# PeihaoChen/WS-MGMap

Hardware: AMD Instinct MI355X
Metric: policy steps/sec (fwd+bwd), CMA batch=8 seq=64 (higher is better)
Workload: dtype bf16

## Files before the change

ws-mgmap_amd/csrc/wsmg_conv_win_wgrad.hip:

```cpp
#include <stdlib.h>

#include "wsmg_conv_tile.h"

namespace {

struct WinWgradArgs {
  const bf16_t* x;
  const bf16_t* dy;
  float* dw;
  int64_t slab;
  int B, H, W, OH, OW, tiles_y, tiles_x, groups;
  unsigned x_bytes, dy_bytes;
};

constexpr int K = 8, S = 2, P = 3, TH = 5, TW = 25;
constexpr int WC = (TW - 1) * S + K;
constexpr int PC = WC / S;
constexpr int PITCH = 192;
constexpr int XROW = S * PC * PITCH;
constexpr int X_BYTES = TH * XROW;
constexpr int NPX = 128;
constexpr int D_BYTES = NPX * PITCH;
constexpr int DPER = NPX * 8 / 256;

__global__ __launch_bounds__(256, 2) void conv_win_wgrad_kernel(WinWgradArgs a) {
  extern __shared__ __attribute__((aligned(16))) unsigned char lds[];
  unsigned char* const xs = lds;
  unsigned char* const ds = lds + X_BYTES;
  const int tid = threadIdx.x, lane = tid & 63, wave = tid >> 6;
  const int xcd = blockIdx.x & 7, li_ = blockIdx.x >> 3;
  const int ky = li_ & 7, grp = xcd + 8 * (li_ >> 3);
  const int tpi = a.tiles_y * a.tiles_x;
  const int ntiles = a.B * tpi;
  const __amdgpu_buffer_rsrc_t xr = make_rsrc(a.x, a.x_bytes), dr = make_rsrc(a.dy, a.dy_bytes);

  constexpr int XPER2 = 2 * TH;
  const int wc0 = tid >> 3, pch = tid & 7;
  const bool has1 = tid < (WC - 32) * 8;
  const int xl0 = ((wc0 & 1) * PC + (wc0 >> 1)) * PITCH + pch * 16;
  const int xl1 = xl0 + 16 * PITCH;
  int doff[DPER];
#pragma unroll
  for (int j = 0; j < DPER; ++j) {
    const int q = wc0 + 32 * j;
    const int qr = (q * 41) >> 10;
    doff[j] = q < TH * TW ? ((qr * a.OW + q - qr * TW) * 64) * 2 + pch * 16 : -1;
  }
  u32x4 rx[XPER2], rd[DPER];
  auto gload = [&](int tile) {
    const int b = tile / tpi, t = tile - b * tpi;
    const int ty = t / a.tiles_x;
    const int oy0 = ty * TH, ox0 = (t - ty * a.tiles_x) * TW;
    const int ix0 = ox0 * S - P, iyb = oy0 * S - P + ky;
    const bool live = tile < ntiles;
    const int c0 = ix0 + wc0, c1 = c0 + 32;
    const bool ok0 = (unsigned)c0 < (unsigned)a.W, ok1 = has1 && (unsigned)c1 < (unsigned)a.W;
    const int cb0 = c0 * 128 + pch * 16, cb1 = cb0 + 32 * 128;
#pragma unroll
    for (int j = 0; j < TH; ++j) {
      const int iy = iyb + j * S;
      const bool rowok = live && (unsigned)iy < (unsigned)a.H;
      const int base = ((b * a.H + iy) * a.W) * 128;
      rx[2 * j] = buf_load16(xr, (rowok && ok0) ? base + cb0 : (int)0x80000000);
      rx[2 * j + 1] = buf_load16(xr, (rowok && ok1) ? base + cb1 : (int)0x80000000);
    }
    const bool whole = live && oy0 + TH <= a.OH && ox0 + TW <= a.OW;
    const int dbase = (((b * a.OH + oy0) * a.OW + ox0) * 64) * 2;
#pragma unroll
    for (int j = 0; j < DPER; ++j) {
      bool ok = whole && doff[j] >= 0;
      if (!whole && live && doff[j] >= 0) {
        const int q = wc0 + 32 * j, qr = (q * 41) >> 10;
        ok = oy0 + qr < a.OH && ox0 + q - qr * TW < a.OW;
      }
      rd[j] = buf_load16(dr, ok ? dbase + doff[j] : (int)0x80000000);
    }
  };
  auto lstore = [&]() {
#pragma unroll
    for (int j = 0; j < TH; ++j) {
      *reinterpret_cast<u32x4*>(xs + j * XROW + xl0) = rx[2 * j];
      if (has1) *reinterpret_cast<u32x4*>(xs + j * XROW + xl1) = rx[2 * j + 1];
    }
#pragma unroll
    for (int j = 0; j < DPER; ++j) *reinterpret_cast<u32x4*>(ds + (wc0 + 32 * j) * PITCH + pch * 16) = rd[j];
  };

  const int li = lane & 15, q4 = li >> 2, p4 = li & 3;
  const int half16 = (lane >> 4) & 1, h = lane >> 5;
  const int chan_off = (half16 * 16 + p4 * 4) * 2;
  const int l0 = 8 * h + q4;
  auto xoff = [&](int c, int s2) {
    int p = 16 * c + l0 + 4 * s2;
    p = p < TH * TW ? p : TH * TW - 1;
    const int jr = (p * 41) >> 10;
    return jr * XROW + (p - jr * TW) * PITCH + chan_off;
  };
  const unsigned char* const a_base = ds + (8 * h + q4) * PITCH + chan_off;
  const int kx0 = 2 * wave;
  const int tapoff0 = ((kx0 & 1) * PC + (kx0 >> 1)) * PITCH, tapoff1 = (((kx0 + 1) & 1) * PC + ((kx0 + 1) >> 1)) * PITCH;

  f32x16 acc[2][4];
#pragma unroll
  for (int t = 0; t < 2; ++t)
#pragma unroll
    for (int v = 0; v < 4; ++v)
#pragma unroll
      for (int g = 0; g < 16; ++g) acc[t][v][g] = 0.f;

  int tile = grp;
  if (tile >= ntiles) return;
  gload(tile);
  lstore();
  __syncthreads();
  struct Frag { bf16x8 a[2], b[4]; };
  auto fload = [&](int c, Frag& f) {
#pragma unroll
    for (int t = 0; t < 2; ++t) {
      const bf16x4 l = tr_read(a_base + 64 * t + (16 * c) * PITCH), hh = tr_read(a_base + 64 * t + (16 * c + 4) * PITCH);
      f.a[t] = __builtin_shufflevector(l, hh, 0, 1, 2, 3, 4, 5, 6, 7);
    }
    const int x0 = xoff(c, 0), x1 = xoff(c, 1);
#pragma unroll
    for (int v = 0; v < 4; ++v) {
      const int to = (v >> 1) ? tapoff1 : tapoff0;
      const bf16x4 l = tr_read(xs + x0 + to + 64 * (v & 1)), hh = tr_read(xs + x1 + to + 64 * (v & 1));
      f.b[v] = __builtin_shufflevector(l, hh, 0, 1, 2, 3, 4, 5, 6, 7);
    }
  };
  for (; tile < ntiles; tile += a.groups) {
    gload(tile + a.groups);
    Frag cur, nxt;
    fload(0, cur);
#pragma unroll
    for (int c = 0; c < 8; ++c) {
      __builtin_amdgcn_sched_barrier(0);
      if (c + 1 < 8) fload(c + 1, nxt);
#pragma unroll
      for (int v = 0; v < 4; ++v)
#pragma unroll
        for (int t = 0; t < 2; ++t) acc[t][v] = __builtin_amdgcn_mfma_f32_32x32x16_bf16(cur.a[t], cur.b[v], acc[t][v], 0, 0, 0);
      if (c + 1 < 8) {
#pragma unroll
        for (int i = 0; i < 4; ++i) {
          __builtin_amdgcn_sched_group_barrier(0x008, 1, 0);
          __builtin_amdgcn_sched_group_barrier(0x100, 2, 0);
          __builtin_amdgcn_sched_group_barrier(0x008, 1, 0);
          __builtin_amdgcn_sched_group_barrier(0x100, 1, 0);
        }
      }
      __builtin_amdgcn_sched_barrier(0);
      if (c + 1 < 8) cur = nxt;
    }
    __syncthreads();
    lstore();
    __syncthreads();
  }

  const int r = lane & 31;
#pragma unroll
  for (int v = 0; v < 4; ++v) {
    const int tap = ky * K + kx0 + (v >> 1);
    const int ci = 32 * (v & 1) + r;
#pragma unroll
    for (int t = 0; t < 2; ++t)
#pragma unroll
      for (int g = 0; g < 16; ++g) {
        const int co = 32 * t + (g & 3) + 8 * (g >> 2) + 4 * h;
        float* const q = a.dw + (size_t)grp * a.slab + ((size_t)co * (K * K) + tap) * 64 + ci;
        if (a.slab) *q = acc[t][v][g];
        else atomicAdd(q, acc[t][v][g]);
      }
  }
}

}

static bool winw_fits(int B, int H, int W, int Cin, int Cout, int KH, int KW, int stride, int pad, int OH, int OW) {
  if (Cin != 64 || Cout != 64 || KH != 8 || KW != 8 || stride != 2 || pad != 3) return false;
  return !((size_t)B * H * W * 128 >= (1ull << 31) || (size_t)B * OH * OW * 128 >= (1ull << 31));
}
static int winw_groups(int B, int OH, int OW) {
  const int ntiles = B * ((OH + TH - 1) / TH) * ((OW + TW - 1) / TW);
  int groups = 64;
  if (groups > ntiles) groups = ntiles;
  return (groups + 7) / 8 * 8;
}

int wsmg_conv_win_wgrad_splits(int B, int H, int W, int Cin, int Cout, int KH, int KW, int stride, int pad, int OH, int OW) {
  return winw_fits(B, H, W, Cin, Cout, KH, KW, stride, pad, OH, OW) ? winw_groups(B, OH, OW) : 0;
}

int wsmg_conv_win_wgrad_bf16(const void* x, const void* dy, float* dw_ohwi, long long slab_floats, int B, int H, int W, int Cin, int Cout,
                             int KH, int KW, int stride, int pad, int OH, int OW, hipStream_t s) {
  if (!winw_fits(B, H, W, Cin, Cout, KH, KW, stride, pad, OH, OW)) return WSMG_EINVAL;
  WinWgradArgs a{(const bf16_t*)x, (const bf16_t*)dy, dw_ohwi, (int64_t)slab_floats, B, H, W, OH, OW, (OH + TH - 1) / TH, (OW + TW - 1) / TW, 0,
                 (unsigned)((size_t)B * H * W * 128), (unsigned)((size_t)B * OH * OW * 128)};
  const int groups = winw_groups(B, OH, OW);
  a.groups = groups;
  static bool attr = false;
  if (!attr) {
    hipError_t e = hipFuncSetAttribute(reinterpret_cast<const void*>(conv_win_wgrad_kernel), hipFuncAttributeMaxDynamicSharedMemorySize,
                                       X_BYTES + D_BYTES);
    if (e != hipSuccess) return (int)e;
    attr = true;
  }
  hipLaunchKernelGGL(conv_win_wgrad_kernel, dim3((unsigned)(8 * groups)), dim3(256), X_BYTES + D_BYTES, s, a);
  WSMG_RETURN_LAUNCH();
}
```

Before: 51600.

## Restructure window wgrad kernel: 512-thread blocks sharing x rows, double-buffered LDS pipeline

Each block now runs 8 waves covering two kernel rows (ky and ky+2), so the staged input rows are shared and the grid shrinks from 8 to 4 blocks per group. The LDS layout is split into channel planes with padding in place of a 192-byte pitch. A double-buffered LDS scheme interleaves the next tile's global loads and LDS stores with the MFMA loop, cutting the per-tile pair of barriers to one. The cost is higher LDS use per block and heavier scheduling constraints, which may lower occupancy. Blocks that have no tile no longer exit early when slab mode is on, so they still write their zero slab.

```diff
diff --git a/ws-mgmap_amd/csrc/wsmg_conv_win_wgrad.hip b/ws-mgmap_amd/csrc/wsmg_conv_win_wgrad.hip
--- a/ws-mgmap_amd/csrc/wsmg_conv_win_wgrad.hip
+++ b/ws-mgmap_amd/csrc/wsmg_conv_win_wgrad.hip
@@ -16,74 +16,74 @@
 constexpr int K = 8, S = 2, P = 3, TH = 5, TW = 25;
 constexpr int WC = (TW - 1) * S + K;
 constexpr int PC = WC / S;
-constexpr int PITCH = 192;
-constexpr int XROW = S * PC * PITCH;
-constexpr int X_BYTES = TH * XROW;
+constexpr int WR = TH + 1;
+constexpr int ENT = 64;
+constexpr int XCH = PC * ENT + 64;
+constexpr int XPAR = 2 * XCH;
+constexpr int XROW = S * XPAR;
+constexpr int X_BYTES = WR * XROW;
 constexpr int NPX = 128;
-constexpr int D_BYTES = NPX * PITCH;
-constexpr int DPER = NPX * 8 / 256;
-
-__global__ __launch_bounds__(256, 2) void conv_win_wgrad_kernel(WinWgradArgs a) {
+constexpr int DCH = NPX * ENT + 64;
+constexpr int D_BYTES = 2 * DCH;
+constexpr int PARK = X_BYTES + D_BYTES;
+constexpr int BUF = PARK + 64 * 16;
+constexpr int LDS_BYTES = 2 * BUF;
+constexpr int NPIECE = WR + 2;
+constexpr int OOB = (int)0x80000000;
+
+__global__ __launch_bounds__(512) void conv_win_wgrad_kernel(WinWgradArgs a) {
   extern __shared__ __attribute__((aligned(16))) unsigned char lds[];
-  unsigned char* const xs = lds;
-  unsigned char* const ds = lds + X_BYTES;
-  const int tid = threadIdx.x, lane = tid & 63, wave = tid >> 6;
+  const int tid = threadIdx.x, lane = tid & 63, wave = __builtin_amdgcn_readfirstlane(tid >> 6);
   const int xcd = blockIdx.x & 7, li_ = blockIdx.x >> 3;
-  const int ky = li_ & 7, grp = xcd + 8 * (li_ >> 3);
+  const int role = li_ & 3, grp = xcd + 8 * (li_ >> 2);
+  const int ky_lo = (role & 1) + 4 * (role >> 1);
   const int tpi = a.tiles_y * a.tiles_x;
   const int ntiles = a.B * tpi;
   const __amdgpu_buffer_rsrc_t xr = make_rsrc(a.x, a.x_bytes), dr = make_rsrc(a.dy, a.dy_bytes);
 
-  constexpr int XPER2 = 2 * TH;
-  const int wc0 = tid >> 3, pch = tid & 7;
-  const bool has1 = tid < (WC - 32) * 8;
-  const int xl0 = ((wc0 & 1) * PC + (wc0 >> 1)) * PITCH + pch * 16;
-  const int xl1 = xl0 + 16 * PITCH;
-  int doff[DPER];
-#pragma unroll
-  for (int j = 0; j < DPER; ++j) {
-    const int q = wc0 + 32 * j;
+  const bool hasx = wave < 7;
+  const int wc = tid >> 3, pch = tid & 7;
+  const int plane = pch >> 2, pbyte = (pch & 3) * 16;
+  const int xl = hasx ? (wc & 1) * XPAR + plane * XCH + (wc >> 1) * ENT + pbyte : PARK + lane * 16;
+  const int xrs = hasx ? XROW : 0;
+  int dl[2], doff[2];
+#pragma unroll
+  for (int j = 0; j < 2; ++j) {
+    const int q = wc + 64 * j;
     const int qr = (q * 41) >> 10;
+    dl[j] = X_BYTES + plane * DCH + q * ENT + pbyte;
     doff[j] = q < TH * TW ? ((qr * a.OW + q - qr * TW) * 64) * 2 + pch * 16 : -1;
   }
-  u32x4 rx[XPER2], rd[DPER];
-  auto gload = [&](int tile) {
+  int t_row0 = 0, t_bH = 0, t_cb = 0, t_dbase = 0;
+  bool t_okx = false, t_okd[2] = {false, false};
+  auto prep = [&](int tile) {
     const int b = tile / tpi, t = tile - b * tpi;
     const int ty = t / a.tiles_x;
     const int oy0 = ty * TH, ox0 = (t - ty * a.tiles_x) * TW;
-    const int ix0 = ox0 * S - P, iyb = oy0 * S - P + ky;
     const bool live = tile < ntiles;
-    const int c0 = ix0 + wc0, c1 = c0 + 32;
-    const bool ok0 = (unsigned)c0 < (unsigned)a.W, ok1 = has1 && (unsigned)c1 < (unsigned)a.W;
-    const int cb0 = c0 * 128 + pch * 16, cb1 = cb0 + 32 * 128;
-#pragma unroll
-    for (int j = 0; j < TH; ++j) {
-      const int iy = iyb + j * S;
-      const bool rowok = live && (unsigned)iy < (unsigned)a.H;
-      const int base = ((b * a.H + iy) * a.W) * 128;
-      rx[2 * j] = buf_load16(xr, (rowok && ok0) ? base + cb0 : (int)0x80000000);
-      rx[2 * j + 1] = buf_load16(xr, (rowok && ok1) ? base + cb1 : (int)0x80000000);
-    }
-    const bool whole = live && oy0 + TH <= a.OH && ox0 + TW <= a.OW;
-    const int dbase = (((b * a.OH + oy0) * a.OW + ox0) * 64) * 2;
-#pragma unroll
-    for (int j = 0; j < DPER; ++j) {
-      bool ok = whole && doff[j] >= 0;
-      if (!whole && live && doff[j] >= 0) {
-        const int q = wc0 + 32 * j, qr = (q * 41) >> 10;
-        ok = oy0 + qr < a.OH && ox0 + q - qr * TW < a.OW;
-      }
-      rd[j] = buf_load16(dr, ok ? dbase + doff[j] : (int)0x80000000);
-    }
-  };
-  auto lstore = [&]() {
-#pragma unroll
-    for (int j = 0; j < TH; ++j) {
-      *reinterpret_cast<u32x4*>(xs + j * XROW + xl0) = rx[2 * j];
-      if (has1) *reinterpret_cast<u32x4*>(xs + j * XROW + xl1) = rx[2 * j + 1];
-    }
-#pragma unroll
-    for (int j = 0; j < DPER; ++j) *reinterpret_cast<u32x4*>(ds + (wc0 + 32 * j) * PITCH + pch * 16) = rd[j];
+    const int c0 = ox0 * S - P + wc;
+    t_okx = hasx && live && (unsigned)c0 < (unsigned)a.W;
+    t_cb = c0 * 128 + pch * 16;
+    t_bH = b * a.H;
+    t_row0 = oy0 * S - P + ky_lo;
+    t_dbase = (((b * a.OH + oy0) * a.OW + ox0) * 64) * 2;
+#pragma unroll
+    for (int j = 0; j < 2; ++j) {
+      const int q = wc + 64 * j, qr = (q * 41) >> 10;
+      t_okd[j] = live && doff[j] >= 0 && oy0 + qr < a.OH && ox0 + q - qr * TW < a.OW;
+    }
+  };
+  auto loadp = [&](int p) -> u32x4 {
+    if (p < WR) {
+      const int iy = t_row0 + p * S;
+      const bool ok = t_okx && (unsigned)iy < (unsigned)a.H;
+      return buf_load16(xr, ok ? ((t_bH + iy) * a.W) * 128 + t_cb : OOB);
+    }
+    return buf_load16(dr, t_okd[p - WR] ? t_dbase + doff[p - WR] : OOB);
+  };
+  u32x4 rp[NPIECE];
+  auto storep = [&](int p, int buf) {
+    *reinterpret_cast<u32x4*>(lds + buf + (p < WR ? xl + p * xrs : dl[p - WR])) = rp[p];
   };
 
   const int li = lane & 15, q4 = li >> 2, p4 = li & 3;
@@ -94,11 +94,11 @@
     int p = 16 * c + l0 + 4 * s2;
     p = p < TH * TW ? p : TH * TW - 1;
     const int jr = (p * 41) >> 10;
-    return jr * XROW + (p - jr * TW) * PITCH + chan_off;
-  };
-  const unsigned char* const a_base = ds + (8 * h + q4) * PITCH + chan_off;
-  const int kx0 = 2 * wave;
-  const int tapoff0 = ((kx0 & 1) * PC + (kx0 >> 1)) * PITCH, tapoff1 = (((kx0 + 1) & 1) * PC + ((kx0 + 1) >> 1)) * PITCH;
+    return jr * XROW + (p - jr * TW) * ENT;
+  };
+  const int a_off = X_BYTES + l0 * ENT + chan_off;
+  const int khalf = wave >> 2, wq = wave & 3;
+  const int x_off = khalf * XROW + wq * ENT + chan_off;
 
   f32x16 acc[2][4];
 #pragma unroll
@@ -109,55 +109,87 @@
       for (int g = 0; g < 16; ++g) acc[t][v][g] = 0.f;
 
   int tile = grp;
-  if (tile >= ntiles) return;
-  gload(tile);
-  lstore();
+  if (tile >= ntiles && !a.slab) return;
+
+  struct Frag { bf16x8 a[2], b[4]; };
+  auto fload = [&](int buf, int c, Frag& f) {
+    const unsigned char* const ab = lds + buf + a_off + (16 * c) * ENT;
+#pragma unroll
+    for (int t = 0; t < 2; ++t) {
+      const bf16x4 l = tr_read(ab + t * DCH), hh = tr_read(ab + t * DCH + 4 * ENT);
+      f.a[t] = __builtin_shufflevector(l, hh, 0, 1, 2, 3, 4, 5, 6, 7);
+    }
+    const unsigned char* const x0 = lds + buf + x_off + xoff(c, 0);
+    const unsigned char* const x1 = lds + buf + x_off + xoff(c, 1);
+#pragma unroll
+    for (int v = 0; v < 4; ++v) {
+      const int to = (v >> 1) * XPAR + (v & 1) * XCH;
+      const bf16x4 l = tr_read(x0 + to), hh = tr_read(x1 + to);
+      f.b[v] = __builtin_shufflevector(l, hh, 0, 1, 2, 3, 4, 5, 6, 7);
+    }
+  };
+
+  prep(tile);
+#pragma unroll
+  for (int p = 0; p < NPIECE; ++p) rp[p] = loadp(p);
+#pragma unroll
+  for (int p = 0; p < NPIECE; ++p) storep(p, 0);
+  prep(tile + a.groups);
+#pragma unroll
+  for (int p = 0; p < NPIECE; ++p) rp[p] = loadp(p);
   __syncthreads();
-  struct Frag { bf16x8 a[2], b[4]; };
-  auto fload = [&](int c, Frag& f) {
-#pragma unroll
-    for (int t = 0; t < 2; ++t) {
-      const bf16x4 l = tr_read(a_base + 64 * t + (16 * c) * PITCH), hh = tr_read(a_base + 64 * t + (16 * c + 4) * PITCH);
-      f.a[t] = __builtin_shufflevector(l, hh, 0, 1, 2, 3, 4, 5, 6, 7);
-    }
-    const int x0 = xoff(c, 0), x1 = xoff(c, 1);
-#pragma unroll
-    for (int v = 0; v < 4; ++v) {
-      const int to = (v >> 1) ? tapoff1 : tapoff0;
-      const bf16x4 l = tr_read(xs + x0 + to + 64 * (v & 1)), hh = tr_read(xs + x1 + to + 64 * (v & 1));
-      f.b[v] = __builtin_shufflevector(l, hh, 0, 1, 2, 3, 4, 5, 6, 7);
-    }
-  };
+  Frag cur;
+  fload(0, 0, cur);
+  int bo = 0;
   for (; tile < ntiles; tile += a.groups) {
-    gload(tile + a.groups);
-    Frag cur, nxt;
-    fload(0, cur);
+    const int bn = BUF - bo;
+    prep(tile + 2 * a.groups);
 #pragma unroll
     for (int c = 0; c < 8; ++c) {
+      Frag nxt;
       __builtin_amdgcn_sched_barrier(0);
-      if (c + 1 < 8) fload(c + 1, nxt);
+      if (c == 7) {
+        __syncthreads();
+        __builtin_amdgcn_sched_barrier(0);
+        fload(bn, 0, nxt);
+      } else {
+        fload(bo, c + 1, nxt);
+        storep(c, bn);
+        rp[c] = loadp(c);
+        if (c == 6) {
+          storep(7, bn);
+          rp[7] = loadp(7);
+        }
+      }
 #pragma unroll
       for (int v = 0; v < 4; ++v)
 #pragma unroll
         for (int t = 0; t < 2; ++t) acc[t][v] = __builtin_amdgcn_mfma_f32_32x32x16_bf16(cur.a[t], cur.b[v], acc[t][v], 0, 0, 0);
-      if (c + 1 < 8) {
-#pragma unroll
-        for (int i = 0; i < 4; ++i) {
-          __builtin_amdgcn_sched_group_barrier(0x008, 1, 0);
-          __builtin_amdgcn_sched_group_barrier(0x100, 2, 0);
-          __builtin_amdgcn_sched_group_barrier(0x008, 1, 0);
-          __builtin_amdgcn_sched_group_barrier(0x100, 1, 0);
-        }
-      }
+#pragma unroll
+      for (int i = 0; i < 3; ++i) {
+        __builtin_amdgcn_sched_group_barrier(0x008, 1, 0);
+        __builtin_amdgcn_sched_group_barrier(0x100, 2, 0);
+        __builtin_amdgcn_sched_group_barrier(0x008, 1, 0);
+        __builtin_amdgcn_sched_group_barrier(0x100, 1, 0);
+      }
+      __builtin_amdgcn_sched_group_barrier(0x008, 1, 0);
+      __builtin_amdgcn_sched_group_barrier(0x100, 3, 0);
+      if (c < 6) {
+        __builtin_amdgcn_sched_group_barrier(0x200, 1, 0);
+        __builtin_amdgcn_sched_group_barrier(0x020, 1, 0);
+      } else if (c == 6) {
+        __builtin_amdgcn_sched_group_barrier(0x200, 2, 0);
+        __builtin_amdgcn_sched_group_barrier(0x020, 2, 0);
+      }
+      __builtin_amdgcn_sched_group_barrier(0x008, 1, 0);
       __builtin_amdgcn_sched_barrier(0);
-      if (c + 1 < 8) cur = nxt;
-    }
-    __syncthreads();
-    lstore();
-    __syncthreads();
+      cur = nxt;
+    }
+    bo = bn;
   }
 
   const int r = lane & 31;
+  const int ky = ky_lo + 2 * khalf, kx0 = 2 * wq;
 #pragma unroll
   for (int v = 0; v < 4; ++v) {
     const int tap = ky * K + kx0 + (v >> 1);
@@ -200,11 +232,10 @@
   a.groups = groups;
   static bool attr = false;
   if (!attr) {
-    hipError_t e = hipFuncSetAttribute(reinterpret_cast<const void*>(conv_win_wgrad_kernel), hipFuncAttributeMaxDynamicSharedMemorySize,
-                                       X_BYTES + D_BYTES);
+    hipError_t e = hipFuncSetAttribute(reinterpret_cast<const void*>(conv_win_wgrad_kernel), hipFuncAttributeMaxDynamicSharedMemorySize, LDS_BYTES);
     if (e != hipSuccess) return (int)e;
     attr = true;
   }
-  hipLaunchKernelGGL(conv_win_wgrad_kernel, dim3((unsigned)(8 * groups)), dim3(256), X_BYTES + D_BYTES, s, a);
+  hipLaunchKernelGGL(conv_win_wgrad_kernel, dim3((unsigned)(4 * groups)), dim3(512), LDS_BYTES, s, a);
   WSMG_RETURN_LAUNCH();
 }
```

New measurement: 52260, median of 6. +1.3%, better.
